# anihcsam/OpenGaussian

Hardware: AMD Instinct MI355X
Metric: fwd+bwd Mpix/s at 1080p, 1M Gaussians (RGB+6-D ins_feat); k-means it/s (higher is better)
Workload: dtype f32; 1 GPU; S1M-1080p RGB(SH3)+depth+alpha (all grads) + 6-ch ins_feat (grad to ins_feat) fwd+bwd, ONE fused 9-channel pass; gaussians=1000000, width=1920, height=1080, views_cycled=8, parallelism=single

## Files before the change

### include/ogs_raster.h

```cpp
#ifndef OGS_RASTER_H
#define OGS_RASTER_H

#include <stddef.h>
#include <stdint.h>

#ifdef __cplusplus
extern "C" {
#endif

#define OGS_OK 0
#define OGS_ERR_INVALID_ARG (-1)
#define OGS_ERR_HIP (-2)
#define OGS_ERR_UNSUPPORTED (-3)
#define OGS_ERR_SCRATCH_TOO_SMALL (-4)
#define OGS_ERR_DEVICE (-5)

#define OGS_TILE 16
#define OGS_MAX_CHANNELS 12

typedef struct OgsRasterFwdArgs {
    int32_t P;
    int32_t W, H;
    int32_t C;
    int32_t sh_degree;
// ... 81 lines not shown
size_t ogs_raster_geom_tmp_bytes(int32_t P);
size_t ogs_raster_image_bytes(int32_t W, int32_t H);
size_t ogs_raster_image_bytes_grouped(int32_t W, int32_t H, int32_t num_groups);
size_t ogs_raster_binning_tmp_bytes(int64_t num_rendered, int32_t W, int32_t H);
size_t ogs_raster_backward_tmp_bytes(int32_t P);
size_t ogs_raster_sorted_bytes(int64_t num_rendered, int32_t C);
size_t ogs_raster_quad_list_bytes(int64_t num_rendered);

int ogs_raster_forward_geometry(const OgsRasterFwdArgs* args, void* stream, int64_t* num_rendered_host);

int ogs_raster_forward_render(const OgsRasterFwdArgs* args, int64_t num_rendered, void* stream);

int ogs_raster_read_num_rendered_async(const OgsRasterFwdArgs* args, void* stream, uint32_t* host_pinned);
int ogs_raster_forward_render_deferred(const OgsRasterFwdArgs* args, int64_t capacity, void* stream);

size_t ogs_raster_tiny_max_points(void);
int ogs_raster_forward_tiny(const OgsRasterFwdArgs* args, void* stream);

size_t ogs_raster_tile_sort_capacity(int32_t level);

int ogs_raster_forward_reblend(const OgsRasterFwdArgs* args, void* stream);

int ogs_raster_compact_kept(int32_t W, int32_t H, int32_t C, const void* image_buffer, const void* sorted_rec,
                            const void* quad_list, void* new_image_buffer, void* new_sorted_rec, void* new_quad_list,
                            void* stream);

typedef struct OgsGroupStatsArgs {
    const int32_t* labels;
    int32_t num_labels;
    float alpha_threshold;
// ... 40 lines not shown
```

### opengaussian_amd/_lib.py

```python
from __future__ import annotations

import ctypes as C
import os

_HERE = os.path.dirname(os.path.abspath(__file__))
LIB_PATH = os.environ.get("OGS_LIB_PATH") or os.path.join(_HERE, "lib", "libogs_hip.so")

_f32p = C.POINTER(C.c_float)
_vp = C.c_void_p


class OgsRasterFwdArgs(C.Structure):
    _fields_ = [
        ("P", C.c_int32), ("W", C.c_int32), ("H", C.c_int32), ("C", C.c_int32),
        ("sh_degree", C.c_int32), ("sh_coeffs", C.c_int32),
        ("tanfovx", C.c_float), ("tanfovy", C.c_float), ("scale_modifier", C.c_float),
        ("prefiltered", C.c_int32), ("debug", C.c_int32),
        ("bg", _vp), ("means3D", _vp), ("colors_precomp", _vp), ("shs", _vp), ("opacities", _vp),
        ("scales", _vp), ("rotations", _vp), ("cov3D_precomp", _vp),
        ("viewmatrix", _vp), ("projmatrix", _vp), ("campos", _vp),
        ("out_color", _vp), ("out_depth", _vp), ("out_alpha", _vp), ("radii", _vp),
        ("geom_buffer", _vp), ("geom_tmp", _vp), ("image_buffer", _vp), ("point_list", _vp),
        ("binning_tmp", _vp), ("sorted_rec", _vp), ("quad_list", _vp), ("group_ids", _vp), ("num_groups", C.c_int32),
        ("full_binning", C.c_int32),
# ... 68 lines not shown
SIGNATURES = {
    "ogs_version": (C.c_int, []),
    "ogs_last_error": (C.c_char_p, []),
    "ogs_raster_geom_bytes": (C.c_size_t, [C.c_int32, C.c_int32]),
    "ogs_raster_geom_tmp_bytes": (C.c_size_t, [C.c_int32]),
    "ogs_raster_image_bytes": (C.c_size_t, [C.c_int32, C.c_int32]),
    "ogs_raster_image_bytes_grouped": (C.c_size_t, [C.c_int32, C.c_int32, C.c_int32]),
    "ogs_raster_binning_tmp_bytes": (C.c_size_t, [C.c_int64, C.c_int32, C.c_int32]),
    "ogs_raster_backward_tmp_bytes": (C.c_size_t, [C.c_int32]),
    "ogs_raster_sorted_bytes": (C.c_size_t, [C.c_int64, C.c_int32]),
    "ogs_raster_quad_list_bytes": (C.c_size_t, [C.c_int64]),
    "ogs_raster_forward_geometry": (C.c_int, [C.POINTER(OgsRasterFwdArgs), _vp, C.POINTER(C.c_int64)]),
    "ogs_raster_forward_render": (C.c_int, [C.POINTER(OgsRasterFwdArgs), C.c_int64, _vp]),
    "ogs_raster_read_num_rendered_async": (C.c_int, [C.POINTER(OgsRasterFwdArgs), _vp, _vp]),
    "ogs_raster_forward_render_deferred": (C.c_int, [C.POINTER(OgsRasterFwdArgs), C.c_int64, _vp]),
    "ogs_raster_stats_image_bytes": (C.c_size_t, [C.c_int32, C.c_int32, C.c_int32]),
    "ogs_raster_stats_tmp_bytes": (C.c_size_t, [C.c_int32, C.c_int32, C.c_int32]),
    "ogs_raster_forward_group_stats": (C.c_int, [C.POINTER(OgsRasterFwdArgs), C.POINTER(OgsGroupStatsArgs), C.c_int64, _vp]),
    "ogs_raster_backward": (C.c_int, [C.POINTER(OgsRasterBwdArgs), _vp]),
    "ogs_raster_tiny_max_points": (C.c_size_t, []),
    "ogs_raster_tile_sort_capacity": (C.c_size_t, [C.c_int32]),
    "ogs_raster_forward_tiny": (C.c_int, [C.POINTER(OgsRasterFwdArgs), _vp]),
    "ogs_raster_forward_reblend": (C.c_int, [C.POINTER(OgsRasterFwdArgs), _vp]),
    "ogs_raster_compact_kept": (C.c_int, [C.c_int32, C.c_int32, C.c_int32, _vp, _vp, _vp, _vp, _vp, _vp, _vp]),
    "ogs_mark_visible": (C.c_int, [C.c_int32, _vp, _vp, _vp, _vp, _vp]),
    "ogs_sh_grad_from_views": (C.c_int, [C.c_int32, C.c_int32, C.c_int32, C.c_int32, _vp, _vp, _vp, _vp, _vp]),
    "ogs_raster_export_binning": (C.c_int, [C.POINTER(OgsRasterFwdArgs), C.c_int64, _vp, _vp, _vp, _vp]),
    "ogs_selftest_wave_fold16": (C.c_int, [_vp, _vp, _vp]),
    "ogs_selftest_mfma_rank1": (C.c_int, [_vp, _vp, _vp, C.c_int32, _vp, _vp, _vp]),
    "ogs_selftest_tile_order": (C.c_int, [_vp, C.c_int64, _vp, _vp]),
# ... 161 lines not shown
```

### opengaussian_amd/csrc/capi.hip

```cpp
#include <stdarg.h>
#include <stdlib.h>
#include <string.h>

#include <map>
#include <mutex>
#include <string>
#include <vector>

#include "ogs_common.h"

namespace ogs {

static thread_local char g_err[512] = "";

void set_error(const char* fmt, ...) {
    va_list ap;
    va_start(ap, fmt);
    vsnprintf(g_err, sizeof(g_err), fmt, ap);
    va_end(ap);
}

namespace {
struct ProfRec { const char* name; hipEvent_t start, stop; };
int g_prof_mode = 0;
// ... 135 lines not shown
    out->opacities = raw->opacity;
    out->scales = raw->scaling;
    out->rotations = raw->rotation;
    if (a->P == 0) {
        out->shs = out->scales = out->rotations = a->bg;
    }
    return OGS_OK;
}

}

using namespace ogs;

extern "C" {

int ogs_version(void) { return 407; }

int ogs_check_async_status(void) { return check_async_status("ogs_check_async_status"); }

int ogs_prof_enable(int on) {
    std::lock_guard<std::mutex> lk(g_prof_mu);
    for (auto& r : g_prof) { g_event_pool.push_back(r.start); g_event_pool.push_back(r.stop); }
    g_prof.clear();
    g_prof_mode = on;
    return OGS_OK;
}

int ogs_prof_filter(const char* prefix) {
    std::lock_guard<std::mutex> lk(g_prof_mu);
    if (!prefix || strlen(prefix) >= sizeof(g_prof_prefix)) { set_error("prof_filter: prefix NULL or longer than %zu", sizeof(g_prof_prefix) - 1); return OGS_ERR_INVALID_ARG; }
    strcpy(g_prof_prefix, prefix);
// ... 113 lines not shown
    if (P == 0) return OGS_OK;
    if (!raw) { set_error("model_activate: raw == NULL"); return OGS_ERR_INVALID_ARG; }
    if ((scales && !raw->scaling) || (rotations && !raw->rotation) || (opacities && !raw->opacity) ||
        (shs && (M < 1 || !raw->features_dc || (M > 1 && !raw->features_rest)))) {
        set_error("model_activate: an output is requested whose raw input is NULL (M=%d)", M); return OGS_ERR_INVALID_ARG;
    }
    return launch_model_activate(P, M, *raw, scales, rotations, opacities, shs, static_cast<hipStream_t>(stream_));
}

int ogs_raster_read_num_rendered_async(const OgsRasterFwdArgs* a, void* stream_, uint32_t* host_pinned) {
    if (!a || !host_pinned) { set_error("read_num_rendered_async: NULL pointer"); return OGS_ERR_INVALID_ARG; }
    if (a->P == 0) { *host_pinned = 0; return OGS_OK; }
    const GeomTmp gt = GeomTmp::carve(a->geom_tmp, a->P);
    OGS_HIP_CHECK(hipMemcpyAsync(host_pinned, gt.num_rendered, sizeof(uint32_t), hipMemcpyDeviceToHost,
                                 static_cast<hipStream_t>(stream_)));
    return OGS_OK;
}

static int render_impl(const OgsRasterFwdArgs* a, int64_t D, bool deferred, hipStream_t s,
                       const OgsGroupStatsArgs* stats = nullptr) {
    int rc = validate_fwd(a, stats == nullptr);
    if (rc != OGS_OK) return rc;
    if (!a->image_buffer) { set_error("image_buffer == NULL"); return OGS_ERR_INVALID_ARG; }
    if (a->bwd_clear && !stats && (((uintptr_t)a->bwd_clear | a->bwd_clear_bytes) & 15u) != 0) {
        set_error("bwd_clear / bwd_clear_bytes must be multiples of 16"); return OGS_ERR_INVALID_ARG;
    }
    const int G = num_groups_of(a->num_groups);
    const ImageState is = stats ? ImageState::carve_stats(a->image_buffer, a->W, a->H, G)
                                : ImageState::carve(a->image_buffer, a->W, a->H, G);
    const int gx = (a->W + kTile - 1) / kTile, gy = (a->H + kTile - 1) / kTile;
// ... 1 lines not shown
    if (tiles >= (1ll << 31)) { set_error("%d groups x %d tiles exceed 2^31 virtual tiles", G, gx * gy); return OGS_ERR_UNSUPPORTED; }
    const GeomState gs = GeomState::carve(a->geom_buffer, a->P > 0 ? a->P : 1, a->C);
    const bool per_tile = per_tile_depth_order(*a);
    bool order_ready = false;
    if (D > 0) {
        if (!a->point_list || !a->binning_tmp) { set_error("point_list / binning_tmp == NULL with num_rendered=%lld", (long long)D); return OGS_ERR_INVALID_ARG; }
        if (D >= (1ll << 31)) { set_error("num_rendered=%lld exceeds 2^31", (long long)D); return OGS_ERR_UNSUPPORTED; }
        const GeomTmp gt = GeomTmp::carve(a->geom_tmp, a->P);
        const BinTmp bt = BinTmp::carve(a->binning_tmp, D);
        const int bits = bit_length((uint32_t)(tiles - 1));
        const int passes = bits == 0 ? 1 : (bits + 7) / 8;
        const int per = bits == 0 ? 1 : (bits + passes - 1) / passes;
        uint32_t* vbuf[2];
        vbuf[passes & 1] = a->point_list;
        vbuf[(passes & 1) ^ 1] = bt.vals;
        const uint32_t* n_dev = deferred ? gt.num_rendered : nullptr;
        const bool cull = a->full_binning == 0;
        const bool zero_in_dup = tiles <= (int64_t)a->P;
        rc = launch_duplicate(*a, gs, gt, bt.tile_keys[0], vbuf[0], (uint32_t)D, cull, !per_tile, s,
                              zero_in_dup ? is.ranges : nullptr, zero_in_dup ? (int)tiles : 0);
        if (rc != OGS_OK) return rc;
        const bool sweep = radix_onesweep_enabled(D);
        int shifts[4], nbits[4];
        for (int p = 0; p < passes; ++p) {
            shifts[p] = p * per;
            nbits[p] = (p == passes - 1) ? (bits == 0 ? 1 : bits - shifts[p]) : per;
        }
        if (passes == 2 && (bits & 1)) {
            nbits[0] = bits / 2; shifts[1] = nbits[0]; nbits[1] = bits - nbits[0];
        }
        if (sweep) {
// ... 285 lines not shown
```

### opengaussian_amd/csrc/ogs_common.h

```cpp
#pragma once

#include <hip/hip_runtime.h>
#include <stdint.h>
#include <stddef.h>
#include <stdio.h>
#include <type_traits>

#include "../../include/ogs_raster.h"
#include "../../include/ogs_model.h"

namespace ogs {

constexpr int kTile = OGS_TILE;
constexpr int kBlock = 256;
constexpr int kWave = 64;
constexpr int kTinyMaxP = 256;
constexpr int kSmallMaxP = 1024;

void set_error(const char* fmt, ...);

#define OGS_HIP_CHECK(expr)                                                              \
    do {                                                                                 \
        hipError_t _e = (expr);                                                          \
        if (_e != hipSuccess) {                                                          \
// ... 174 lines not shown

int exclusive_scan_u32(const uint32_t* in, const uint32_t* gather, uint32_t* out, int64_t n,
                       uint32_t* total, void* tmp, hipStream_t stream, int debug, const uint32_t* n_dev = nullptr);
constexpr uint32_t kDropKey = 0xFFFFFFFFu;
bool radix_onesweep_enabled(int64_t n);
int radix_sort_begin(const uint32_t* keys, int64_t n, const uint32_t* n_dev, int npass, const int* shifts, const int* bits,
                     void* tmp, hipStream_t stream, int debug, bool drop = false, int items = 0);
int radix_sort_pass(int pass, int npass, const uint32_t* keys_in, const uint32_t* vals_in, uint32_t* keys_out,
                    uint32_t* vals_out, int64_t n, int shift, int bits, void* tmp, hipStream_t stream, int debug,
                    const uint32_t* n_dev = nullptr, bool drop = false, uint32_t* kept_out = nullptr, int items = 0,
                    int spin_limit = -1);
int radix_pass(const uint32_t* keys_in, const uint32_t* vals_in, uint32_t* keys_out, uint32_t* vals_out,
               int64_t n, int shift, int bits, void* tmp, hipStream_t stream, int debug,
               const uint32_t* n_dev = nullptr, bool drop = false, uint32_t* kept_out = nullptr);

struct GeomTmp {
    uint32_t* tiles_touched;
    uint32_t* keys[2];
    uint32_t* order[2];
    uint32_t* offsets;
    uint32_t* num_rendered;
    void* sort_tmp;
    uint32_t* block_sum;
    uint32_t* visible() const { return num_rendered + 1; }
    static GeomTmp carve(void* p, int P) {
        Carver c(p);
        GeomTmp g;
        g.tiles_touched = c.take<uint32_t>(P);
        g.keys[0] = c.take<uint32_t>(P);
        g.keys[1] = c.take<uint32_t>(P);
        g.order[0] = c.take<uint32_t>(P);
        g.order[1] = c.take<uint32_t>(P);
        g.offsets = c.take<uint32_t>(P);
        g.num_rendered = c.take<uint32_t>(64);
        g.sort_tmp = c.take<char>(sort_tmp_bytes(P));
        g.block_sum = c.take<uint32_t>((size_t)(P + kBlock - 1) / kBlock);
        return g;
    }
    static size_t bytes(int P) {
        Carver c(nullptr);
        for (int i = 0; i < 6; ++i) c.take<uint32_t>(P);
        c.take<uint32_t>(64);
        c.take<char>(sort_tmp_bytes(P));
        c.take<uint32_t>((size_t)(P + kBlock - 1) / kBlock);
        return c.off;
    }
};

struct BinTmp {
    uint32_t* tile_keys[2];
    uint32_t* vals;
    uint32_t* kept;
    void* sort_tmp;
    static BinTmp carve(void* p, int64_t D) {
        Carver c(p);
        BinTmp b;
        b.tile_keys[0] = c.take<uint32_t>(D);
        b.tile_keys[1] = c.take<uint32_t>(D);
        b.vals = c.take<uint32_t>(D);
// ... 111 lines not shown
```

### opengaussian_amd/csrc/preprocess_fwd.hip

```cpp
#include "ogs_common.h"
#include "ogs_model_act.h"

namespace ogs {

namespace {

__constant__ const float kC0 = 0.28209479177387814f;
__constant__ const float kC1 = 0.4886025119029199f;
__constant__ const float kC2[5] = {1.0925484305920792f, -1.0925484305920792f, 0.31539156525252005f,
                                   -1.0925484305920792f, 0.5462742152960396f};
__constant__ const float kC3[7] = {-0.5900435899266435f, 2.890611442640554f, -0.4570457994644658f,
                                   0.3731763325901154f, -0.4570457994644658f, 1.445305721320277f,
                                   -0.5900435899266435f};

struct Cam {
    float V[16];
    float M[16];
    float campos[3];
};

template <bool RAW>
__device__ __forceinline__ void cov3d_from_scale_rot(const float* __restrict__ scales,
                                                     const float* __restrict__ rots, int idx, float mod,
                                                     float cov[6]) {
// ... 56 lines not shown
    for (int c = 0; c < 3; ++c) {
        res[c] = res[c] + 0.5f;
        if (res[c] < 0.f) clamped |= 1u << c;
        rgb[c] = fmaxf(res[c], 0.f);
    }
}

template <int C, bool RAW>
__device__ __forceinline__ uint32_t preprocess_one(
    int idx, int W, int H, int sh_degree, int sh_coeffs, float tanfovx, float tanfovy, float focal_x, float focal_y,
    float scale_modifier, const float* __restrict__ means3D, const float* __restrict__ colors_precomp,
    const float* __restrict__ shs, const float* __restrict__ opacities, const float* __restrict__ scales,
    const float* __restrict__ rotations, const float* __restrict__ cov3D_precomp, const float* __restrict__ viewmatrix,
    const float* __restrict__ projmatrix, const float* __restrict__ campos, float4* __restrict__ rec_row,
    uint32_t* __restrict__ clamped_out, int32_t* __restrict__ radii, uint32_t* __restrict__ tiles_touched,
    const int32_t* __restrict__ group_ids, int num_groups, uint32_t* touched_ret = nullptr) {
    constexpr int NV = rec_vec4(C);
    float V[16], M[16];
#pragma unroll
    for (int i = 0; i < 16; ++i) { V[i] = viewmatrix[i]; M[i] = projmatrix[i]; }

    const float x = means3D[3 * idx + 0], y = means3D[3 * idx + 1], z = means3D[3 * idx + 2];
    const float opacity = RAW ? act_opacity(opacities[idx]) : opacities[idx];

    float feat[(C + 3) / 4 * 4];
#pragma unroll
    for (int c = 0; c < (C + 3) / 4 * 4; ++c) feat[c] = 0.f;
    uint32_t clamped = 0;

    int radius = 0;
    uint32_t touched = 0;
    float pxl = 0.f, pyl = 0.f, depth = 0.f, cA = 0.f, cB = 0.f, cC = 0.f;

    const float pvx = V[0] * x + V[4] * y + V[8] * z + V[12];
    const float pvy = V[1] * x + V[5] * y + V[9] * z + V[13];
    const float pvz = V[2] * x + V[6] * y + V[10] * z + V[14];
    bool ok = pvz > 0.2f;
    if (group_ids != nullptr) ok = ok && (uint32_t)group_ids[idx] < (uint32_t)num_groups;
    if (ok) {
        const float hx = M[0] * x + M[4] * y + M[8] * z + M[12];
        const float hy = M[1] * x + M[5] * y + M[9] * z + M[13];
        const float hw = M[3] * x + M[7] * y + M[11] * z + M[15];
        const float p_w = 1.0f / (hw + 0.0000001f);
        const float projx = hx * p_w, projy = hy * p_w;
        float cov[6];
        if (!RAW && cov3D_precomp != nullptr) {
// ... 46 lines not shown
            auto tr = [](float v) -> int {
                if (!(fabsf(v) < 3.0e38f)) v = 0.f;
                v = fminf(fmaxf(v, -2.0e9f), 2.0e9f);
                return (int)v;
            };
            const int rminx = min(gx, max(0, tr((pxl - rf) / (float)kTile)));
            const int rminy = min(gy, max(0, tr((pyl - rf) / (float)kTile)));
            const int rmaxx = min(gx, max(0, tr((pxl + rf + (float)kTile - 1.0f) / (float)kTile)));
            const int rmaxy = min(gy, max(0, tr((pyl + rf + (float)kTile - 1.0f) / (float)kTile)));
            const int area = (rmaxx - rminx) * (rmaxy - rminy);
            ok = area != 0 && my_radius > 0;
            if (ok) {
                radius = my_radius;
                touched = (uint32_t)area;
                depth = pvz;
            }
        }
    }

    const int coff = shs != nullptr ? 3 : 0;
    if (colors_precomp != nullptr) {
#pragma unroll
        for (int c = 0; c < C; ++c)
            if (c >= coff) feat[c] = colors_precomp[(size_t)idx * (C - coff) + (c - coff)];
    }
    if (shs != nullptr && ok) {
        float rgb[3];
        float cp[3] = {campos[0], campos[1], campos[2]};
        if constexpr (RAW) sh_to_rgb(sh_degree, raw_sh_row(shs, cov3D_precomp, idx, sh_coeffs), x, y, z, cp, rgb, clamped);
        else sh_to_rgb(sh_degree, shs + (size_t)idx * sh_coeffs * 3, x, y, z, cp, rgb, clamped);
        feat[0] = rgb[0]; feat[1] = rgb[1]; feat[2] = rgb[2];
    }

    if (!ok) { pxl = 0.f; pyl = 0.f; cA = cB = cC = 0.f; depth = 0.f; }

    float4* r = rec_row;
    r[0] = make_float4(pxl, pyl, depth, __int_as_float(radius));
    r[1] = make_float4(cA, cB, cC, opacity);
#pragma unroll
    for (int v = 0; v < NV - 2; ++v) r[2 + v] = make_float4(feat[4 * v], feat[4 * v + 1], feat[4 * v + 2], feat[4 * v + 3]);
    clamped_out[idx] = clamped;
    radii[idx] = radius;
    if (tiles_touched) tiles_touched[idx] = touched;
    if (touched_ret) *touched_ret = touched;
    return ok ? __float_as_uint(depth) : 0xFFFFFFFFu;
}

template <int C, bool RAW>
__global__ __launch_bounds__(kBlock) void preprocess_kernel(
    int P, int W, int H, int sh_degree, int sh_coeffs, float tanfovx, float tanfovy, float focal_x, float focal_y,
    float scale_modifier, const float* __restrict__ means3D, const float* __restrict__ colors_precomp,
    const float* __restrict__ shs, const float* __restrict__ opacities, const float* __restrict__ scales,
    const float* __restrict__ rotations, const float* __restrict__ cov3D_precomp, const float* __restrict__ viewmatrix,
    const float* __restrict__ projmatrix, const float* __restrict__ campos, float4* __restrict__ rec,
    uint32_t* __restrict__ clamped_out, int32_t* __restrict__ radii, uint32_t* __restrict__ tiles_touched,
    uint32_t* __restrict__ depth_keys, uint32_t* __restrict__ order, const int32_t* __restrict__ group_ids,
    int num_groups, uint32_t* __restrict__ block_sum) {
    constexpr int NV = rec_vec4(C);
    __shared__ float4 s_rec[kBlock * NV];
    __shared__ uint32_t s_wave_sum[kBlock / kWave];
    const int tid = threadIdx.x;
    const int idx = blockIdx.x * kBlock + tid;
    uint32_t touched = 0;
    if (idx < P) {
        depth_keys[idx] = preprocess_one<C, RAW>(idx, W, H, sh_degree, sh_coeffs, tanfovx, tanfovy, focal_x, focal_y, scale_modifier,
                                            means3D, colors_precomp, shs, opacities, scales, rotations, cov3D_precomp, viewmatrix,
                                            projmatrix, campos, s_rec + tid * NV, clamped_out, radii, tiles_touched, group_ids,
                                            num_groups, &touched);
        if (order) order[idx] = (uint32_t)idx;
    }
    if (block_sum != nullptr) {
        uint32_t t = touched;
#pragma unroll
        for (int d = kWave / 2; d >= 1; d >>= 1) t += __shfl_down(t, d, kWave);
        if ((tid & (kWave - 1)) == 0) s_wave_sum[tid / kWave] = t;
    }
    __syncthreads();
    if (block_sum != nullptr && tid == 0) {
        uint32_t t = 0;
#pragma unroll
        for (int w = 0; w < kBlock / kWave; ++w) t += s_wave_sum[w];
        block_sum[blockIdx.x] = t;
    }
    const size_t row0 = (size_t)blockIdx.x * kBlock;
    const int n4 = min(kBlock, P - (int)row0) * NV;
    float4* __restrict__ out = rec + row0 * NV;
    for (int e = tid; e < n4; e += kBlock) out[e] = s_rec[e];
}

template <int C, bool RAW>
__global__ __launch_bounds__(kTinyMaxP) void tiny_geometry_kernel(
    int P, int W, int H, int sh_degree, int sh_coeffs, float tanfovx, float tanfovy, float focal_x, float focal_y,
    float scale_modifier, const float* __restrict__ means3D, const float* __restrict__ colors_precomp,
    const float* __restrict__ shs, const float* __restrict__ opacities, const float* __restrict__ scales,
    const float* __restrict__ rotations, const float* __restrict__ cov3D_precomp, const float* __restrict__ viewmatrix,
    const float* __restrict__ projmatrix, const float* __restrict__ campos, float4* __restrict__ rec,
    uint32_t* __restrict__ clamped_out, int32_t* __restrict__ radii, uint32_t* __restrict__ order) {
// ... 63 lines not shown
#pragma unroll
    for (int w = 0; w < kSmallMaxP / kWave; ++w) {
        const uint32_t t = s_wave[w];
        if (w < wave) before += t;
        total += t;
    }
    if (idx < P) offsets[idx] = before + incl - v;
    if (idx == 0) { num_rendered[0] = total; num_rendered[1] = (uint32_t)P; }
}

template <int NV>
__global__ __launch_bounds__(kBlock) void duplicate_kernel(int P_cap, const uint32_t* __restrict__ n_visible, int W, int H,
                                                           const float4* __restrict__ rec,
                                                           const uint32_t* __restrict__ order,
                                                           const uint32_t* __restrict__ offsets,
                                                           const uint32_t* __restrict__ tiles_touched,
                                                           const uint32_t* __restrict__ block_base,
                                                           uint32_t* __restrict__ tile_keys,
                                                           uint32_t* __restrict__ vals, uint32_t capacity,
                                                           const int32_t* __restrict__ group_ids, bool drop_unreachable,
                                                           uint2* __restrict__ zero_ranges, int n_zero) {
    __shared__ uint32_t s_wave_sum[kBlock / kWave];
    __shared__ uint32_t s_off[kBlock];
    __shared__ uint32_t s_gid[kBlock];
    __shared__ uint32_t s_rect[kBlock];
    __shared__ uint32_t s_first, s_total;
    __shared__ uint32_t s_key0[kBlock];
    __shared__ float4 s_ctr[kBlock];
    __shared__ float4 s_con[kBlock];
    const int tid = threadIdx.x;
    const int r = blockIdx.x * kBlock + tid;
    if (zero_ranges != nullptr && r < n_zero) zero_ranges[r] = make_uint2(0u, 0u);
    const int P = n_visible ? min(P_cap, (int)*n_visible) : P_cap;
    if ((int)blockIdx.x * kBlock >= P) return;
    const int gx = (W + kTile - 1) / kTile, gy = (H + kTile - 1) / kTile;
    uint32_t off = 0, cnt = 0, gid = 0, rect = 1u << 24, key0 = 0, touched = 0;
    float4 ctr = make_float4(0.f, 0.f, 0.f, 0.f);
    float4 con = make_float4(1.f, 1.f, 0.f, 0.f);
    int wide_x0 = 0, wide_x1 = 0, wide_y0 = 0, wide_y1 = 0;
    if (r < P) {
        gid = order ? order[r] : (uint32_t)r;
        if (block_base != nullptr) touched = tiles_touched[r];
        else off = offsets[r];
        if (group_ids != nullptr) key0 = (uint32_t)max(group_ids[gid], 0) * (uint32_t)(gx * gy);
        const float4 a = rec[(size_t)gid * NV];
        const int radius = __float_as_int(a.w);
        if (radius > 0) {
            const float4 b = rec[(size_t)gid * NV + 1];
            ctr = make_float4(a.x, a.y, -(__logf(255.0f * b.w) + kThrMargin), b.y);
            con = make_float4(b.x, b.z, -b.y / b.x, -b.y / b.z);
            const float rf = (float)radius;
            auto tr = [](float v) -> int {
                if (!(fabsf(v) < 3.0e38f)) v = 0.f;
                v = fminf(fmaxf(v, -2.0e9f), 2.0e9f);
                return (int)v;
            };
            const int rminx = min(gx, max(0, tr((a.x - rf) / (float)kTile)));
            const int rminy = min(gy, max(0, tr((a.y - rf) / (float)kTile)));
            const int rmaxx = min(gx, max(0, tr((a.x + rf + (float)kTile - 1.0f) / (float)kTile)));
            const int rmaxy = min(gy, max(0, tr((a.y + rf + (float)kTile - 1.0f) / (float)kTile)));
            const int w = rmaxx - rminx, h = rmaxy - rminy;
            if (w > 0 && h > 0) {
                cnt = (uint32_t)(w * h);
                rect = (uint32_t)rminx | ((uint32_t)rminy << 12) | ((uint32_t)min(w, 255) << 24);
                if (w > 255) { wide_x0 = rminx; wide_x1 = rmaxx; wide_y0 = rminy; wide_y1 = rmaxy; }
            }
        }
    }
    uint32_t before = 0;
    if (block_base != nullptr) {
        const int lane = tid & (kWave - 1);
        uint32_t incl = touched;
#pragma unroll
        for (int d = 1; d < kWave; d <<= 1) {
            const uint32_t o = __shfl_up(incl, d, kWave);
            if (lane >= d) incl += o;
        }
        if (lane == kWave - 1) s_wave_sum[tid / kWave] = incl;
        before = incl - touched;
        if (tid == 0) s_first = block_base[blockIdx.x];
    } else if (tid == 0) {
// ... 43 lines not shown
        if (o < capacity) {
            const uint32_t tx = (rc & 0xFFFu) + col, ty = (rc >> 12 & 0xFFFu) + row;
            const uint32_t key = s_key0[lo] + ty * (uint32_t)gx + tx;
            const float4 c = s_ctr[lo];
            const float4 k = s_con[lo];
            const float X0 = (float)(tx * kTile), Y0 = (float)(ty * kTile);
            const float m = max_power_in_box(k.x, c.w, k.y, k.z, k.w, c.x - X0 - 15.f, c.x - X0, c.y - Y0 - 15.f, c.y - Y0);
            const bool reach = m >= c.z;
            tile_keys[o] = (drop_unreachable && !reach) ? kDropKey : key;
            vals[o] = g | ((reach ? 1u : 0u) << kReachBit);
        }
    }
}

constexpr int kOffsThreads = 1024, kOffsItems = 8, kOffsChunk = kOffsThreads * kOffsItems;
__global__ __launch_bounds__(kOffsThreads) void block_offsets_kernel(uint32_t* __restrict__ block_sum, int nb,
                                                                     uint32_t* __restrict__ total_out) {
    __shared__ uint32_t s_val[kOffsChunk];
    __shared__ uint32_t s_wave_sum[kOffsThreads / kWave];
    const int tid = threadIdx.x, lane = tid & (kWave - 1), wave = tid / kWave;
    uint32_t carry = 0;
    for (int c0 = 0; c0 < nb; c0 += kOffsChunk) {
        const int n = min(kOffsChunk, nb - c0);
#pragma unroll
        for (int k = 0; k < kOffsItems; ++k) {
            const int e = k * kOffsThreads + tid;
            s_val[e] = e < n ? block_sum[c0 + e] : 0u;
        }
        __syncthreads();
        uint32_t v[kOffsItems], sum = 0;
#pragma unroll
        for (int k = 0; k < kOffsItems; ++k) { v[k] = s_val[tid * kOffsItems + k]; sum += v[k]; }
        uint32_t incl = sum;
#pragma unroll
        for (int d = 1; d < kWave; d <<= 1) {
            const uint32_t o = __shfl_up(incl, d, kWave);
            if (lane >= d) incl += o;
        }
        if (lane == kWave - 1) s_wave_sum[wave] = incl;
        __syncthreads();
        uint32_t run = carry + incl - sum, total = 0;
#pragma unroll
        for (int w = 0; w < kOffsThreads / kWave; ++w) {
            const uint32_t t = s_wave_sum[w];
            if (w < wave) run += t;
            total += t;
        }
#pragma unroll
        for (int k = 0; k < kOffsItems; ++k) {
            const int e = tid * kOffsItems + k;
            if (e < n) block_sum[c0 + e] = run;
            run += v[k];
        }
        carry += total;
        __syncthreads();
    }
    if (tid == 0) total_out[0] = carry;
}

__global__ __launch_bounds__(kBlock) void mark_visible_kernel(int P, const float* __restrict__ means3D,
                                                              const float* __restrict__ V,
                                                              uint8_t* __restrict__ present) {
    const int idx = blockIdx.x * kBlock + threadIdx.x;
    if (idx >= P) return;
    const float x = means3D[3 * idx], y = means3D[3 * idx + 1], z = means3D[3 * idx + 2];
    const float pvz = V[2] * x + V[6] * y + V[10] * z + V[14];
    present[idx] = pvz > 0.2f ? 1 : 0;
}

__global__ __launch_bounds__(kBlock) void model_activate_kernel(int P, int M, const float* __restrict__ features_dc,
                                                                const float* __restrict__ features_rest,
                                                                const float* __restrict__ scaling,
// ... 23 lines not shown
            shs[row0 * L + e] = i < 3 ? features_dc[(row0 + g) * 3 + i] : features_rest[(row0 + g) * Lr + (i - 3)];
        }
    }
}

template <int C, bool RAW>
int launch_preprocess_c(const OgsRasterFwdArgs& a, const GeomState& gs, const GeomTmp& gt, hipStream_t s) {
    const float focal_x = (float)a.W / (2.0f * a.tanfovx);
    const float focal_y = (float)a.H / (2.0f * a.tanfovy);
    const int grid = (a.P + kBlock - 1) / kBlock;
    static constexpr const char* const kNames[4] = {"preprocess_kernel<3>", "preprocess_kernel<6>", "preprocess_kernel<9>", "preprocess_kernel<12>"};
    static constexpr const char* const kRawNames[4] = {"preprocess_kernel<3, raw>", "preprocess_kernel<6, raw>", "preprocess_kernel<9, raw>", "preprocess_kernel<12, raw>"};
    OGS_LAUNCH_NAMED(chan_name<C>(RAW ? kRawNames : kNames), (preprocess_kernel<C, RAW>), dim3(grid), dim3(kBlock), 0, s, a.P, a.W, a.H, a.sh_degree, a.sh_coeffs,
                       a.tanfovx, a.tanfovy, focal_x, focal_y, a.scale_modifier, a.means3D, a.colors_precomp, a.shs,
                       a.opacities, a.scales, a.rotations, a.cov3D_precomp, a.viewmatrix, a.projmatrix, a.campos,
                       gs.rec, gs.clamped, a.radii, gt.tiles_touched, gt.keys[0],
                       per_tile_depth_order(a) ? (uint32_t*)nullptr : gt.order[0], a.num_groups > 1 ? a.group_ids : (const int32_t*)nullptr, a.num_groups,
                       block_sum_offsets(a) ? gt.block_sum : (uint32_t*)nullptr);
    OGS_LAUNCH_CHECK(a.debug, s);
    return OGS_OK;
}

template <int C, bool RAW>
int launch_tiny_geometry_c(const OgsRasterFwdArgs& a, const GeomState& gs, uint32_t* order, hipStream_t s) {
    const float focal_x = (float)a.W / (2.0f * a.tanfovx);
    const float focal_y = (float)a.H / (2.0f * a.tanfovy);
    OGS_LAUNCH_NAMED(RAW ? "tiny_geometry_kernel<C, raw>" : "tiny_geometry_kernel<C>", (tiny_geometry_kernel<C, RAW>), dim3(1), dim3(kTinyMaxP), 0, s, a.P, a.W, a.H, a.sh_degree, a.sh_coeffs, a.tanfovx,
               a.tanfovy, focal_x, focal_y, a.scale_modifier, a.means3D, a.colors_precomp, a.shs, a.opacities, a.scales,
               a.rotations, a.cov3D_precomp, a.viewmatrix, a.projmatrix, a.campos, gs.rec, gs.clamped, a.radii, order);
    OGS_LAUNCH_CHECK(a.debug, s);
    return OGS_OK;
}

// ... 47 lines not shown

int launch_duplicate(const OgsRasterFwdArgs& a, const GeomState& gs, const GeomTmp& gt, uint32_t* tile_keys,
                     uint32_t* vals, uint32_t capacity, bool drop_unreachable, bool depth_order, hipStream_t s, uint2* zero_ranges,
                     int n_zero) {
    const uint32_t* base = (!depth_order && block_sum_offsets(a)) ? gt.block_sum : nullptr;
    if (n_zero > a.P) { set_error("duplicate: %d ranges to clear with %d threads", n_zero, a.P); return OGS_ERR_INVALID_ARG; }
    const int grid = (a.P + kBlock - 1) / kBlock;
    const int32_t* grp = a.num_groups > 1 ? a.group_ids : nullptr;
    if ((a.W + kTile - 1) / kTile > 4095 || (a.H + kTile - 1) / kTile > 4095) {
        set_error("image %dx%d exceeds 4095 tiles per side", a.W, a.H);
        return OGS_ERR_UNSUPPORTED;
    }
    const uint32_t* order = depth_order ? gt.order[0] : nullptr;
    const uint32_t* n_visible = depth_order ? gt.visible() : nullptr;
    switch (rec_vec4(a.C)) {
        case 3: OGS_LAUNCH(duplicate_kernel<3>, dim3(grid), dim3(kBlock), 0, s, a.P, n_visible, a.W, a.H, gs.rec, order, gt.offsets, gt.tiles_touched, base, tile_keys, vals, capacity, grp, drop_unreachable, zero_ranges, n_zero); break;
        case 4: OGS_LAUNCH(duplicate_kernel<4>, dim3(grid), dim3(kBlock), 0, s, a.P, n_visible, a.W, a.H, gs.rec, order, gt.offsets, gt.tiles_touched, base, tile_keys, vals, capacity, grp, drop_unreachable, zero_ranges, n_zero); break;
        case 5: OGS_LAUNCH(duplicate_kernel<5>, dim3(grid), dim3(kBlock), 0, s, a.P, n_visible, a.W, a.H, gs.rec, order, gt.offsets, gt.tiles_touched, base, tile_keys, vals, capacity, grp, drop_unreachable, zero_ranges, n_zero); break;
        default: set_error("unsupported record size"); return OGS_ERR_UNSUPPORTED;
    }
    OGS_LAUNCH_CHECK(a.debug, s);
    return OGS_OK;
}

int launch_mark_visible(int P, const float* means3D, const float* viewmatrix, uint8_t* present, hipStream_t s) {
    const int grid = (P + kBlock - 1) / kBlock;
    OGS_LAUNCH(mark_visible_kernel, dim3(grid), dim3(kBlock), 0, s, P, means3D, viewmatrix, present);
    OGS_LAUNCH_CHECK(0, s);
    return OGS_OK;
}

}
```

### opengaussian_amd/rasterizer.py

```python
from __future__ import annotations

import ctypes as C
import functools
import os
from typing import NamedTuple, Optional

import torch
from torch import nn

from . import _lib
from ._lib import OgsRasterBwdArgs, OgsRasterFwdArgs, OgsRawModel, OgsRawModelGrads, check, ptr

SUPPORTED_CHANNELS = (3, 6, 9, 12)
BACKWARD_CHANNELS = (3, 6, 9)
TINY_MAX_P = 256
_DEBUG_KEEP_BWD_TMP = None
_LAST_NUM_RENDERED: dict = {}
_HINT_WINDOW = 32
PASS_STATS = {"blocking": 0, "deferred": 0, "overflow": 0, "tiny": 0, "tiny_rerendered_for_backward": 0, "reblend": 0,
              "raw_model": 0}


def _hint_capacity(key):
    hist = _LAST_NUM_RENDERED.get(key)
    if not hist:
        return None
    return int(max(hist) * 1.25) + 4096


def _hint_record(key, D):
    from collections import deque
# ... 178 lines not shown
        pinned, ev = _readback_slot(dev)
        check(lib.ogs_raster_read_num_rendered_async(C.byref(a), stream, pinned.data_ptr()),
              "ogs_raster_read_num_rendered_async")
        ev.record()
        PASS_STATS["deferred"] += 1
        point_list, bin_tmp, sorted_rec, quad_list = alloc_render(cap)
        check(lib.ogs_raster_forward_render_deferred(C.byref(a), cap, stream), "ogs_raster_forward_render_deferred")
        ev.synchronize()
        check(lib.ogs_check_async_status(), "ogs_check_async_status")
        D = int(pinned.item()) & 0xFFFFFFFF
        if D > cap:
            PASS_STATS["overflow"] += 1
            point_list, bin_tmp, sorted_rec, quad_list = alloc_render(D)
            check(lib.ogs_raster_forward_render(C.byref(a), D, stream), "ogs_raster_forward_render")
    _hint_record(key, D)
    return geom, image, point_list, sorted_rec, quad_list, D


class _RasterizeGaussians(torch.autograd.Function):
    @staticmethod
    def forward(ctx, means3D, means2D, sh, colors_precomp, opacities, scales, rotations, cov3Ds_precomp,
                raster_settings: GaussianRasterizationSettings, geom_channels: int = 0, sh_rgb_sink=None,
                group_ids=None, num_groups: int = 1, keep_sink=None, force_streaming: bool = False):
        rs = raster_settings
        ctx.geom_channels = int(geom_channels)
        ctx.sh_rgb_sink = sh_rgb_sink
        ctx.set_materialize_grads(False)
        G = max(int(num_groups), 1)
        ctx.num_groups = G
        if G > 1:
# ... 936 lines not shown
```

Baseline: 1492 Mpix/s.

## Tighten per-Gaussian tile rectangles to opacity-threshold ellipse in preprocess

Preprocess now computes a tighter tile rectangle per Gaussian from the ellipse where alpha exceeds the 1/255 threshold, stores it packed in a new emit_rect buffer, and block-sums both the emitted count and the original touched count. The duplicate kernel reads the precomputed rectangle instead of recomputing it from the radius, and the sort runs only over the emitted count, so fewer tile/key pairs are duplicated, sorted and rendered. Capacity still uses the conservative touched total. It costs extra per-Gaussian math and an 8-byte write per point, plus a debug readback helper.

```diff
diff --git a/include/ogs_raster.h b/include/ogs_raster.h
--- a/include/ogs_raster.h
+++ b/include/ogs_raster.h
@@ -119,6 +119,8 @@
 int ogs_raster_read_num_rendered_async(const OgsRasterFwdArgs* args, void* stream, uint32_t* host_pinned);
 int ogs_raster_forward_render_deferred(const OgsRasterFwdArgs* args, int64_t capacity, void* stream);
 
+int ogs_raster_read_num_emitted(const OgsRasterFwdArgs* args, void* stream, uint32_t* host);
+
 size_t ogs_raster_tiny_max_points(void);
 int ogs_raster_forward_tiny(const OgsRasterFwdArgs* args, void* stream);
 
diff --git a/opengaussian_amd/_lib.py b/opengaussian_amd/_lib.py
--- a/opengaussian_amd/_lib.py
+++ b/opengaussian_amd/_lib.py
@@ -106,6 +106,7 @@
     "ogs_raster_forward_render": (C.c_int, [C.POINTER(OgsRasterFwdArgs), C.c_int64, _vp]),
     "ogs_raster_read_num_rendered_async": (C.c_int, [C.POINTER(OgsRasterFwdArgs), _vp, _vp]),
     "ogs_raster_forward_render_deferred": (C.c_int, [C.POINTER(OgsRasterFwdArgs), C.c_int64, _vp]),
+    "ogs_raster_read_num_emitted": (C.c_int, [C.POINTER(OgsRasterFwdArgs), _vp, C.POINTER(C.c_uint32)]),
     "ogs_raster_stats_image_bytes": (C.c_size_t, [C.c_int32, C.c_int32, C.c_int32]),
     "ogs_raster_stats_tmp_bytes": (C.c_size_t, [C.c_int32, C.c_int32, C.c_int32]),
     "ogs_raster_forward_group_stats": (C.c_int, [C.POINTER(OgsRasterFwdArgs), C.POINTER(OgsGroupStatsArgs), C.c_int64, _vp]),
diff --git a/opengaussian_amd/csrc/capi.hip b/opengaussian_amd/csrc/capi.hip
--- a/opengaussian_amd/csrc/capi.hip
+++ b/opengaussian_amd/csrc/capi.hip
@@ -173,7 +173,7 @@
 
 extern "C" {
 
-int ogs_version(void) { return 407; }
+int ogs_version(void) { return 408; }
 
 int ogs_check_async_status(void) { return check_async_status("ogs_check_async_status"); }
 
@@ -317,6 +317,18 @@
     const GeomTmp gt = GeomTmp::carve(a->geom_tmp, a->P);
     OGS_HIP_CHECK(hipMemcpyAsync(host_pinned, gt.num_rendered, sizeof(uint32_t), hipMemcpyDeviceToHost,
                                  static_cast<hipStream_t>(stream_)));
+    return OGS_OK;
+}
+
+int ogs_raster_read_num_emitted(const OgsRasterFwdArgs* a, void* stream_, uint32_t* host) {
+    if (!a || !host) { set_error("read_num_emitted: NULL pointer"); return OGS_ERR_INVALID_ARG; }
+    *host = 0;
+    if (a->P == 0) return OGS_OK;
+    if (!a->geom_tmp) { set_error("read_num_emitted: geom_tmp == NULL"); return OGS_ERR_INVALID_ARG; }
+    const GeomTmp gt = GeomTmp::carve(a->geom_tmp, a->P);
+    hipStream_t s = static_cast<hipStream_t>(stream_);
+    OGS_HIP_CHECK(hipMemcpyAsync(host, block_sum_offsets(*a) ? gt.emitted() : gt.num_rendered, sizeof(uint32_t), hipMemcpyDeviceToHost, s));
+    OGS_HIP_CHECK(hipStreamSynchronize(s));
     return OGS_OK;
 }
 
@@ -348,7 +360,7 @@
         uint32_t* vbuf[2];
         vbuf[passes & 1] = a->point_list;
         vbuf[(passes & 1) ^ 1] = bt.vals;
-        const uint32_t* n_dev = deferred ? gt.num_rendered : nullptr;
+        const uint32_t* n_dev = block_sum_offsets(*a) ? gt.emitted() : deferred ? gt.num_rendered : nullptr;
         const bool cull = a->full_binning == 0;
         const bool zero_in_dup = tiles <= (int64_t)a->P;
         rc = launch_duplicate(*a, gs, gt, bt.tile_keys[0], vbuf[0], (uint32_t)D, cull, !per_tile, s,
diff --git a/opengaussian_amd/csrc/ogs_common.h b/opengaussian_amd/csrc/ogs_common.h
--- a/opengaussian_amd/csrc/ogs_common.h
+++ b/opengaussian_amd/csrc/ogs_common.h
@@ -212,6 +212,9 @@
                int64_t n, int shift, int bits, void* tmp, hipStream_t stream, int debug,
                const uint32_t* n_dev = nullptr, bool drop = false, uint32_t* kept_out = nullptr);
 
+constexpr int kBlockSumPad = 8;
+__host__ __device__ constexpr int block_sum_run(int nb) { return (nb + kBlockSumPad - 1) / kBlockSumPad * kBlockSumPad; }
+
 struct GeomTmp {
     uint32_t* tiles_touched;
     uint32_t* keys[2];
@@ -220,7 +223,10 @@
     uint32_t* num_rendered;
     void* sort_tmp;
     uint32_t* block_sum;
+    uint2* emit_rect;
+    static constexpr int kEmittedWord = 2;
     uint32_t* visible() const { return num_rendered + 1; }
+    uint32_t* emitted() const { return num_rendered + kEmittedWord; }
     static GeomTmp carve(void* p, int P) {
         Carver c(p);
         GeomTmp g;
@@ -232,7 +238,8 @@
         g.offsets = c.take<uint32_t>(P);
         g.num_rendered = c.take<uint32_t>(64);
         g.sort_tmp = c.take<char>(sort_tmp_bytes(P));
-        g.block_sum = c.take<uint32_t>((size_t)(P + kBlock - 1) / kBlock);
+        g.block_sum = c.take<uint32_t>(2 * (size_t)block_sum_run((P + kBlock - 1) / kBlock));
+        g.emit_rect = c.take<uint2>(P);
         return g;
     }
     static size_t bytes(int P) {
@@ -240,7 +247,8 @@
         for (int i = 0; i < 6; ++i) c.take<uint32_t>(P);
         c.take<uint32_t>(64);
         c.take<char>(sort_tmp_bytes(P));
-        c.take<uint32_t>((size_t)(P + kBlock - 1) / kBlock);
+        c.take<uint32_t>(2 * (size_t)block_sum_run((P + kBlock - 1) / kBlock));
+        c.take<uint2>(P);
         return c.off;
     }
 };
diff --git a/opengaussian_amd/csrc/preprocess_fwd.hip b/opengaussian_amd/csrc/preprocess_fwd.hip
--- a/opengaussian_amd/csrc/preprocess_fwd.hip
+++ b/opengaussian_amd/csrc/preprocess_fwd.hip
@@ -94,7 +94,8 @@
     const float* __restrict__ rotations, const float* __restrict__ cov3D_precomp, const float* __restrict__ viewmatrix,
     const float* __restrict__ projmatrix, const float* __restrict__ campos, float4* __restrict__ rec_row,
     uint32_t* __restrict__ clamped_out, int32_t* __restrict__ radii, uint32_t* __restrict__ tiles_touched,
-    const int32_t* __restrict__ group_ids, int num_groups, uint32_t* touched_ret = nullptr) {
+    const int32_t* __restrict__ group_ids, int num_groups, uint32_t* touched_ret = nullptr,
+    uint2* __restrict__ emit_rect = nullptr, uint32_t* emitted_ret = nullptr) {
     constexpr int NV = rec_vec4(C);
     float V[16], M[16];
 #pragma unroll
@@ -109,7 +110,8 @@
     uint32_t clamped = 0;
 
     int radius = 0;
-    uint32_t touched = 0;
+    uint32_t touched = 0, emitted = 0;
+    uint2 erect = make_uint2(0u, 0u);
     float pxl = 0.f, pyl = 0.f, depth = 0.f, cA = 0.f, cB = 0.f, cC = 0.f;
 
     const float pvx = V[0] * x + V[4] * y + V[8] * z + V[12];
@@ -186,6 +188,29 @@
                 radius = my_radius;
                 touched = (uint32_t)area;
                 depth = pvz;
+                if (emit_rect != nullptr) {
+                    const float Rr = rf + 17.0f;
+                    const float tmax = (0.5f * (cA + cC) + fabsf(cB)) * (Rr * Rr);
+                    const float t = 2.0f * ((__logf(255.0f * opacity) + kThrMargin) + (1.0e-4f + 1.25e-6f * tmax));
+                    const float dcf = (float)((double)cA * (double)cC - (double)cB * (double)cB);
+                    const float pad = 1.0e-6f * (fmaxf(fabsf(pxl), fabsf(pyl)) + Rr) + 1.0e-3f;
+                    const float hx = sqrtf(t * (cC / dcf)) * 1.00001f + pad;
+                    const float hy = sqrtf(t * (cA / dcf)) * 1.00001f + pad;
+                    int ex0 = rminx, ex1 = rmaxx, ey0 = rminy, ey1 = rmaxy;
+                    const bool ellipse = cA > 0.f && cC > 0.f && dcf > 0.f
+                                         && rmaxx - rminx <= 255;
+                    if (ellipse && t < 0.f) {
+                        ex0 = ex1 = ey0 = ey1 = 0;
+                    } else if (ellipse && hx < 3.0e38f && hy < 3.0e38f) {
+                        ex0 = max(ex0, tr(ceilf((pxl - hx - 15.0f) / (float)kTile)));
+                        ey0 = max(ey0, tr(ceilf((pyl - hy - 15.0f) / (float)kTile)));
+                        ex1 = min(ex1, tr(floorf((pxl + hx) / (float)kTile)) + 1);
+                        ey1 = min(ey1, tr(floorf((pyl + hy) / (float)kTile)) + 1);
+                        if (ex1 <= ex0 || ey1 <= ey0) ex0 = ex1 = ey0 = ey1 = 0;
+                    }
+                    emitted = (uint32_t)((ex1 - ex0) * (ey1 - ey0));
+                    erect = make_uint2((uint32_t)ex0 | ((uint32_t)ex1 << 16), (uint32_t)ey0 | ((uint32_t)ey1 << 16));
+                }
             }
         }
     }
@@ -215,6 +240,7 @@
     radii[idx] = radius;
     if (tiles_touched) tiles_touched[idx] = touched;
     if (touched_ret) *touched_ret = touched;
+    if (emit_rect) { emit_rect[idx] = erect; *emitted_ret = emitted; }
     return ok ? __float_as_uint(depth) : 0xFFFFFFFFu;
 }
 
@@ -227,32 +253,32 @@
     const float* __restrict__ projmatrix, const float* __restrict__ campos, float4* __restrict__ rec,
     uint32_t* __restrict__ clamped_out, int32_t* __restrict__ radii, uint32_t* __restrict__ tiles_touched,
     uint32_t* __restrict__ depth_keys, uint32_t* __restrict__ order, const int32_t* __restrict__ group_ids,
-    int num_groups, uint32_t* __restrict__ block_sum) {
+    int num_groups, uint32_t* __restrict__ block_sum, uint2* __restrict__ emit_rect) {
     constexpr int NV = rec_vec4(C);
     __shared__ float4 s_rec[kBlock * NV];
-    __shared__ uint32_t s_wave_sum[kBlock / kWave];
+    __shared__ uint32_t s_wave_sum[2][kBlock / kWave];
     const int tid = threadIdx.x;
     const int idx = blockIdx.x * kBlock + tid;
-    uint32_t touched = 0;
+    uint32_t touched = 0, emitted = 0;
     if (idx < P) {
         depth_keys[idx] = preprocess_one<C, RAW>(idx, W, H, sh_degree, sh_coeffs, tanfovx, tanfovy, focal_x, focal_y, scale_modifier,
                                             means3D, colors_precomp, shs, opacities, scales, rotations, cov3D_precomp, viewmatrix,
                                             projmatrix, campos, s_rec + tid * NV, clamped_out, radii, tiles_touched, group_ids,
-                                            num_groups, &touched);
+                                            num_groups, &touched, emit_rect, &emitted);
         if (order) order[idx] = (uint32_t)idx;
     }
     if (block_sum != nullptr) {
-        uint32_t t = touched;
-#pragma unroll
-        for (int d = kWave / 2; d >= 1; d >>= 1) t += __shfl_down(t, d, kWave);
-        if ((tid & (kWave - 1)) == 0) s_wave_sum[tid / kWave] = t;
+        uint32_t t = emitted, u = touched;
+#pragma unroll
+        for (int d = kWave / 2; d >= 1; d >>= 1) { t += __shfl_down(t, d, kWave); u += __shfl_down(u, d, kWave); }
+        if ((tid & (kWave - 1)) == 0) { s_wave_sum[0][tid / kWave] = t; s_wave_sum[1][tid / kWave] = u; }
     }
     __syncthreads();
-    if (block_sum != nullptr && tid == 0) {
+    if (block_sum != nullptr && tid < 2) {
         uint32_t t = 0;
 #pragma unroll
-        for (int w = 0; w < kBlock / kWave; ++w) t += s_wave_sum[w];
-        block_sum[blockIdx.x] = t;
+        for (int w = 0; w < kBlock / kWave; ++w) t += s_wave_sum[tid][w];
+        block_sum[tid * block_sum_run((int)gridDim.x) + blockIdx.x] = t;
     }
     const size_t row0 = (size_t)blockIdx.x * kBlock;
     const int n4 = min(kBlock, P - (int)row0) * NV;
@@ -346,7 +372,7 @@
                                                            const float4* __restrict__ rec,
                                                            const uint32_t* __restrict__ order,
                                                            const uint32_t* __restrict__ offsets,
-                                                           const uint32_t* __restrict__ tiles_touched,
+                                                           const uint2* __restrict__ emit_rect,
                                                            const uint32_t* __restrict__ block_base,
                                                            uint32_t* __restrict__ tile_keys,
                                                            uint32_t* __restrict__ vals, uint32_t capacity,
@@ -372,31 +398,40 @@
     int wide_x0 = 0, wide_x1 = 0, wide_y0 = 0, wide_y1 = 0;
     if (r < P) {
         gid = order ? order[r] : (uint32_t)r;
-        if (block_base != nullptr) touched = tiles_touched[r];
-        else off = offsets[r];
         if (group_ids != nullptr) key0 = (uint32_t)max(group_ids[gid], 0) * (uint32_t)(gx * gy);
-        const float4 a = rec[(size_t)gid * NV];
-        const int radius = __float_as_int(a.w);
-        if (radius > 0) {
+        int rminx = 0, rminy = 0, rmaxx = 0, rmaxy = 0;
+        float4 a = make_float4(0.f, 0.f, 0.f, 0.f);
+        if (block_base != nullptr) {
+            const uint2 e = emit_rect[r];
+            rminx = (int)(e.x & 0xFFFFu); rmaxx = (int)(e.x >> 16);
+            rminy = (int)(e.y & 0xFFFFu); rmaxy = (int)(e.y >> 16);
+            touched = (uint32_t)((rmaxx - rminx) * (rmaxy - rminy));
+            if (touched != 0u) a = rec[(size_t)gid * NV];
+        } else {
+            off = offsets[r];
+            a = rec[(size_t)gid * NV];
+            const int radius = __float_as_int(a.w);
+            if (radius > 0) {
+                const float rf = (float)radius;
+                auto tr = [](float v) -> int {
+                    if (!(fabsf(v) < 3.0e38f)) v = 0.f;
+                    v = fminf(fmaxf(v, -2.0e9f), 2.0e9f);
+                    return (int)v;
+                };
+                rminx = min(gx, max(0, tr((a.x - rf) / (float)kTile)));
+                rminy = min(gy, max(0, tr((a.y - rf) / (float)kTile)));
+                rmaxx = min(gx, max(0, tr((a.x + rf + (float)kTile - 1.0f) / (float)kTile)));
+                rmaxy = min(gy, max(0, tr((a.y + rf + (float)kTile - 1.0f) / (float)kTile)));
+            }
+        }
+        const int w = rmaxx - rminx, h = rmaxy - rminy;
+        if (w > 0 && h > 0) {
             const float4 b = rec[(size_t)gid * NV + 1];
             ctr = make_float4(a.x, a.y, -(__logf(255.0f * b.w) + kThrMargin), b.y);
             con = make_float4(b.x, b.z, -b.y / b.x, -b.y / b.z);
-            const float rf = (float)radius;
-            auto tr = [](float v) -> int {
-                if (!(fabsf(v) < 3.0e38f)) v = 0.f;
-                v = fminf(fmaxf(v, -2.0e9f), 2.0e9f);
-                return (int)v;
-            };
-            const int rminx = min(gx, max(0, tr((a.x - rf) / (float)kTile)));
-            const int rminy = min(gy, max(0, tr((a.y - rf) / (float)kTile)));
-            const int rmaxx = min(gx, max(0, tr((a.x + rf + (float)kTile - 1.0f) / (float)kTile)));
-            const int rmaxy = min(gy, max(0, tr((a.y + rf + (float)kTile - 1.0f) / (float)kTile)));
-            const int w = rmaxx - rminx, h = rmaxy - rminy;
-            if (w > 0 && h > 0) {
-                cnt = (uint32_t)(w * h);
-                rect = (uint32_t)rminx | ((uint32_t)rminy << 12) | ((uint32_t)min(w, 255) << 24);
-                if (w > 255) { wide_x0 = rminx; wide_x1 = rmaxx; wide_y0 = rminy; wide_y1 = rmaxy; }
-            }
+            cnt = (uint32_t)(w * h);
+            rect = (uint32_t)rminx | ((uint32_t)rminy << 12) | ((uint32_t)min(w, 255) << 24);
+            if (w > 255) { wide_x0 = rminx; wide_x1 = rmaxx; wide_y0 = rminy; wide_y1 = rmaxy; }
         }
     }
     uint32_t before = 0;
@@ -470,30 +505,42 @@
 }
 
 constexpr int kOffsThreads = 1024, kOffsItems = 8, kOffsChunk = kOffsThreads * kOffsItems;
+static_assert(kOffsItems == 8 && kBlockSumPad == 8, "two uint4 per thread and run");
 __global__ __launch_bounds__(kOffsThreads) void block_offsets_kernel(uint32_t* __restrict__ block_sum, int nb,
                                                                      uint32_t* __restrict__ total_out) {
-    __shared__ uint32_t s_val[kOffsChunk];
     __shared__ uint32_t s_wave_sum[kOffsThreads / kWave];
+    __shared__ uint32_t s_ref_sum[kOffsThreads / kWave];
     const int tid = threadIdx.x, lane = tid & (kWave - 1), wave = tid / kWave;
-    uint32_t carry = 0;
+    const uint32_t* __restrict__ ref_sum = block_sum + block_sum_run(nb);
+    uint32_t carry = 0, ref_total = 0;
     for (int c0 = 0; c0 < nb; c0 += kOffsChunk) {
         const int n = min(kOffsChunk, nb - c0);
+        const int e0 = tid * kOffsItems;
+        uint32_t v[kOffsItems], u[kOffsItems], sum = 0, ref = 0;
+#pragma unroll
+        for (int k = 0; k < kOffsItems; ++k) v[k] = u[k] = 0u;
+        if (e0 < n) {
+            const uint4 a0 = *reinterpret_cast<const uint4*>(block_sum + c0 + e0), a1 = *reinterpret_cast<const uint4*>(block_sum + c0 + e0 + 4);
+            const uint4 r0 = *reinterpret_cast<const uint4*>(ref_sum + c0 + e0), r1 = *reinterpret_cast<const uint4*>(ref_sum + c0 + e0 + 4);
+            v[0] = a0.x; v[1] = a0.y; v[2] = a0.z; v[3] = a0.w; v[4] = a1.x; v[5] = a1.y; v[6] = a1.z; v[7] = a1.w;
+            u[0] = r0.x; u[1] = r0.y; u[2] = r0.z; u[3] = r0.w; u[4] = r1.x; u[5] = r1.y; u[6] = r1.z; u[7] = r1.w;
+        }
 #pragma unroll
         for (int k = 0; k < kOffsItems; ++k) {
-            const int e = k * kOffsThreads + tid;
-            s_val[e] = e < n ? block_sum[c0 + e] : 0u;
-        }
-        __syncthreads();
-        uint32_t v[kOffsItems], sum = 0;
-#pragma unroll
-        for (int k = 0; k < kOffsItems; ++k) { v[k] = s_val[tid * kOffsItems + k]; sum += v[k]; }
+            if (e0 + k >= n) v[k] = u[k] = 0u;
+            sum += v[k];
+            ref += u[k];
+        }
         uint32_t incl = sum;
 #pragma unroll
         for (int d = 1; d < kWave; d <<= 1) {
             const uint32_t o = __shfl_up(incl, d, kWave);
             if (lane >= d) incl += o;
         }
+#pragma unroll
+        for (int d = kWave / 2; d >= 1; d >>= 1) ref += __shfl_down(ref, d, kWave);
         if (lane == kWave - 1) s_wave_sum[wave] = incl;
+        if (lane == 0) s_ref_sum[wave] = ref;
         __syncthreads();
         uint32_t run = carry + incl - sum, total = 0;
 #pragma unroll
@@ -501,17 +548,17 @@
             const uint32_t t = s_wave_sum[w];
             if (w < wave) run += t;
             total += t;
+            ref_total += s_ref_sum[w];
         }
 #pragma unroll
         for (int k = 0; k < kOffsItems; ++k) {
-            const int e = tid * kOffsItems + k;
-            if (e < n) block_sum[c0 + e] = run;
+            if (e0 + k < n) block_sum[c0 + e0 + k] = run;
             run += v[k];
         }
         carry += total;
         __syncthreads();
     }
-    if (tid == 0) total_out[0] = carry;
+    if (tid == 0) { total_out[0] = ref_total; total_out[GeomTmp::kEmittedWord] = carry; }
 }
 
 __global__ __launch_bounds__(kBlock) void mark_visible_kernel(int P, const float* __restrict__ means3D,
@@ -565,9 +612,9 @@
     OGS_LAUNCH_NAMED(chan_name<C>(RAW ? kRawNames : kNames), (preprocess_kernel<C, RAW>), dim3(grid), dim3(kBlock), 0, s, a.P, a.W, a.H, a.sh_degree, a.sh_coeffs,
                        a.tanfovx, a.tanfovy, focal_x, focal_y, a.scale_modifier, a.means3D, a.colors_precomp, a.shs,
                        a.opacities, a.scales, a.rotations, a.cov3D_precomp, a.viewmatrix, a.projmatrix, a.campos,
-                       gs.rec, gs.clamped, a.radii, gt.tiles_touched, gt.keys[0],
+                       gs.rec, gs.clamped, a.radii, block_sum_offsets(a) ? (uint32_t*)nullptr : gt.tiles_touched, gt.keys[0],
                        per_tile_depth_order(a) ? (uint32_t*)nullptr : gt.order[0], a.num_groups > 1 ? a.group_ids : (const int32_t*)nullptr, a.num_groups,
-                       block_sum_offsets(a) ? gt.block_sum : (uint32_t*)nullptr);
+                       block_sum_offsets(a) ? gt.block_sum : (uint32_t*)nullptr, block_sum_offsets(a) ? gt.emit_rect : (uint2*)nullptr);
     OGS_LAUNCH_CHECK(a.debug, s);
     return OGS_OK;
 }
@@ -645,9 +692,9 @@
     const uint32_t* order = depth_order ? gt.order[0] : nullptr;
     const uint32_t* n_visible = depth_order ? gt.visible() : nullptr;
     switch (rec_vec4(a.C)) {
-        case 3: OGS_LAUNCH(duplicate_kernel<3>, dim3(grid), dim3(kBlock), 0, s, a.P, n_visible, a.W, a.H, gs.rec, order, gt.offsets, gt.tiles_touched, base, tile_keys, vals, capacity, grp, drop_unreachable, zero_ranges, n_zero); break;
-        case 4: OGS_LAUNCH(duplicate_kernel<4>, dim3(grid), dim3(kBlock), 0, s, a.P, n_visible, a.W, a.H, gs.rec, order, gt.offsets, gt.tiles_touched, base, tile_keys, vals, capacity, grp, drop_unreachable, zero_ranges, n_zero); break;
-        case 5: OGS_LAUNCH(duplicate_kernel<5>, dim3(grid), dim3(kBlock), 0, s, a.P, n_visible, a.W, a.H, gs.rec, order, gt.offsets, gt.tiles_touched, base, tile_keys, vals, capacity, grp, drop_unreachable, zero_ranges, n_zero); break;
+        case 3: OGS_LAUNCH(duplicate_kernel<3>, dim3(grid), dim3(kBlock), 0, s, a.P, n_visible, a.W, a.H, gs.rec, order, gt.offsets, gt.emit_rect, base, tile_keys, vals, capacity, grp, drop_unreachable, zero_ranges, n_zero); break;
+        case 4: OGS_LAUNCH(duplicate_kernel<4>, dim3(grid), dim3(kBlock), 0, s, a.P, n_visible, a.W, a.H, gs.rec, order, gt.offsets, gt.emit_rect, base, tile_keys, vals, capacity, grp, drop_unreachable, zero_ranges, n_zero); break;
+        case 5: OGS_LAUNCH(duplicate_kernel<5>, dim3(grid), dim3(kBlock), 0, s, a.P, n_visible, a.W, a.H, gs.rec, order, gt.offsets, gt.emit_rect, base, tile_keys, vals, capacity, grp, drop_unreachable, zero_ranges, n_zero); break;
         default: set_error("unsupported record size"); return OGS_ERR_UNSUPPORTED;
     }
     OGS_LAUNCH_CHECK(a.debug, s);
diff --git a/opengaussian_amd/rasterizer.py b/opengaussian_amd/rasterizer.py
--- a/opengaussian_amd/rasterizer.py
+++ b/opengaussian_amd/rasterizer.py
@@ -15,6 +15,7 @@
 BACKWARD_CHANNELS = (3, 6, 9)
 TINY_MAX_P = 256
 _DEBUG_KEEP_BWD_TMP = None
+_DEBUG_EMITTED = None
 _LAST_NUM_RENDERED: dict = {}
 _HINT_WINDOW = 32
 PASS_STATS = {"blocking": 0, "deferred": 0, "overflow": 0, "tiny": 0, "tiny_rerendered_for_backward": 0, "reblend": 0,
@@ -223,6 +224,10 @@
             point_list, bin_tmp, sorted_rec, quad_list = alloc_render(D)
             check(lib.ogs_raster_forward_render(C.byref(a), D, stream), "ogs_raster_forward_render")
     _hint_record(key, D)
+    if _DEBUG_EMITTED is not None:
+        n = C.c_uint32(0)
+        check(lib.ogs_raster_read_num_emitted(C.byref(a), stream, C.byref(n)), "ogs_raster_read_num_emitted")
+        _DEBUG_EMITTED.append((D, int(n.value)))
     return geom, image, point_list, sorted_rec, quad_list, D
 
 
```

Result: faster. 1516 Mpix/s (median of 6 runs) (+1.6%).
